# MuMuJun97/semantic_slam_mapping

Measured on AMD Instinct MI355X. Metric: frames/sec semantic-mapping, 640x480 RGB-D, higher is better.
Workload: dtype u8; 1 GPU; configs[1]: synthetic 640x480 RGB-D + precomputed 12-class masks, 1k frames per GPU, ORB 1000 kp/frame, 5 ref frames, leaf 0.10 m; frames_per_gpu=1000, frames_all_gpus=1000, batch_frames=250, matcher_halo_frames=0, parallelism=single GPU

## Files before the change

semantic_slam_mapping_amd/csrc/kernels_match.hip:

```cpp
#include "ssm_internal.h"

#define MT 512
#define TCH 1024

#define QPL 2
__device__ __forceinline__ uint32_t bcnt_acc(uint32_t x, uint32_t acc)
{
    uint32_t r;
    asm("v_bcnt_u32_b32 %0, %1, %2" : "=v"(r) : "v"(x), "v"(acc));
    return r;
}
__device__ __forceinline__ uint32_t umed3(uint32_t a, uint32_t b, uint32_t c)
{
    uint32_t r;
    asm("v_med3_u32 %0, %1, %2, %3" : "=v"(r) : "v"(a), "v"(b), "v"(c));
    return r;
}
template <int T>
__device__ __forceinline__ void match_pair(const uint8_t* __restrict__ q, int nq, const uint8_t* __restrict__ t, int nt,
                                           double ratio, int cap, ssm_dmatch* __restrict__ out, int32_t* __restrict__ nout,
                                           int32_t* __restrict__ knn_idx, int32_t* __restrict__ knn_dist,
                                           int qb = 0, int qe = -1, int32_t* __restrict__ pend = nullptr, int role = 0)
{
    __shared__ uint4 tr[TCH * 2];
    __shared__ int wcnt[T / 64];
    __shared__ int base;
    const int tid = threadIdx.x, lane = tid & 63, wv = tid >> 6;
    if (qe < 0) qe = nq;
    if (tid == 0) base = role == 2 ? qb : 0;
    for (int q0 = qb; q0 < qe; q0 += T * QPL) {
        uint4 a[QPL], b[QPL]; uint32_t k0[QPL], k1[QPL];
#pragma unroll
        for (int u = 0; u < QPL; u++) {
// ... 90 lines not shown
__global__ void __launch_bounds__(MT / 2)
match_seq_kernel(const uint8_t* __restrict__ desc, const int32_t* __restrict__ nkp, int f0, int R, int hist, double ratio, int cap,
                 ssm_dmatch* __restrict__ out, int32_t* __restrict__ nout, int32_t* __restrict__ pend)
{
    const int f = f0 + blockIdx.y, r = blockIdx.x >> 1, half = blockIdx.x & 1;
    const int cur = hist + f, ref = cur - R + r;
    const int slot = f * R + r;
    const int nq = ref >= 0 ? nkp[ref] : -1, nt = nkp[cur];
    if (nq < 0 || nt < 2) { if (threadIdx.x == 0 && half == 0) nout[slot] = -1; return; }
    const int split = min(nq, (((nq + 1) >> 1) + 63) & ~63);
    match_pair<MT / 2>(desc + (size_t)ref * cap * 32, nq, desc + (size_t)cur * cap * 32, nt, ratio, cap,
                       out + (size_t)slot * cap, nout + slot, nullptr, nullptr, half ? split : 0, half ? nq : split, pend + blockIdx.y * R + r, half + 1);
}
hipError_t k_match_seq(const uint8_t* desc, const int32_t* nkp, int f0, int n, int R, int hist, double ratio, int cap,
                       ssm_dmatch* out, int32_t* nout, int32_t* pend, hipStream_t s)
{
    hipError_t e = hipMemsetAsync(pend, 0xFF, sizeof(int32_t) * (size_t)n * R, s);
    if (e != hipSuccess) return e;
    match_seq_kernel<<<dim3(2 * R, n), MT / 2, 0, s>>>(desc, nkp, f0, R, hist, ratio, cap, out, nout, pend);
    return hipGetLastError();
}

typedef int v4i __attribute__((ext_vector_type(4)));
typedef int v8i __attribute__((ext_vector_type(8)));
typedef float v16f __attribute__((ext_vector_type(16)));
typedef __attribute__((address_space(3))) void* lds_ptr_t;
#define MM_QB 256
#define MM_DB SSM_MATCH_DESC_BYTES
#define MM_KS 4
#define MM_TILE (32 * MM_DB)
#ifndef MM_ABLATE
#define MM_ABLATE 0
#endif

__global__ void __launch_bounds__(256)
match_expand_kernel(const uint8_t* __restrict__ desc, const int32_t* __restrict__ nkp, int row0, int cap, int capT,
                    uint8_t* __restrict__ eq, uint8_t* __restrict__ et)
{
    const int row = row0 + blockIdx.y;
    const int i = blockIdx.x * 256 + threadIdx.x;
    if (i >= capT * 8) return;
    const int r = i & 31, c = (i >> 5) & 7, d = (i >> 8) * 32 + r;
    uint32_t bits = 0;
    if (d < nkp[row]) bits = *reinterpret_cast<const uint32_t*>(desc + ((size_t)row * cap + d) * 32 + 4 * c);
    uint32_t q[4], t[4];
#pragma unroll
    for (int k = 0; k < 4; k++) {
        uint32_t v = (bits >> (8 * k)) & 255u;
        v = (v | (v << 12)) & 0x000F000Fu;
        v = (v | (v << 6)) & 0x03030303u;
        v = (v | (v << 3)) & 0x11111111u;
        q[k] = (v << 3) + 0x22222222u;
        t[k] = (v << 3) ^ 0xAAAAAAAAu;
    }
    const size_t o = (size_t)row * capT * MM_DB + (size_t)i * 16;
    *reinterpret_cast<uint4*>(eq + o) = make_uint4(q[0], q[1], q[2], q[3]);
    *reinterpret_cast<uint4*>(et + o) = make_uint4(t[0], t[1], t[2], t[3]);
}

__device__ __forceinline__ void mm_merge2(uint32_t& a0, uint32_t& a1, uint32_t b0, uint32_t b1)
{
    const uint32_t m = max(a0, b0);
    a0 = min(a0, b0);
    a1 = min(min(m, a1), b1);
}
__device__ __forceinline__ void mm_track(const v16f& acc, uint32_t t32, uint32_t& g0, uint32_t& g1)
{
    float l0 = __builtin_fminf(acc[0], acc[1]), l1 = __builtin_fmaxf(acc[0], acc[1]);
#pragma unroll
    for (int i = 2; i < 16; i++) { l1 = __builtin_amdgcn_fmed3f(acc[i], l0, l1); l0 = __builtin_fminf(acc[i], l0); }
    const uint32_t k0 = (uint32_t)l0, k1 = (uint32_t)l1;
    const uint32_t G0 = ((k0 >> 5) << 16) | ((k0 & 31u) | t32), G1 = ((k1 >> 5) << 16) | ((k1 & 31u) | t32);
    mm_merge2(g0, g1, G0, G1);
}

__global__ void __launch_bounds__(256, 2)
match_mfma_kernel(const uint8_t* __restrict__ eq, const uint8_t* __restrict__ et, const int32_t* __restrict__ nkp,
                  int f0, int n, int R, int hist, int capT, int qblocks, int frames_per_xcd, uint2* __restrict__ knn)
{
    __shared__ __attribute__((aligned(16))) uint4 ring0[MM_TILE / 16];
    __shared__ __attribute__((aligned(16))) uint4 ring1[MM_TILE / 16];
    __shared__ __attribute__((aligned(16))) uint4 ring2[MM_TILE / 16];
    __shared__ __attribute__((aligned(16))) uint4 ring3[MM_TILE / 16];
    const int Y = R * qblocks, xcd = blockIdx.x & 7, j = blockIdx.x >> 3;
    const int frame = xcd * frames_per_xcd + j / Y, y = j % Y;
    if (frame >= n) return;
    const int r = y / qblocks, qb = y - r * qblocks;
    const int f = f0 + frame, cur = hist + f, ref = cur - R + r;
    const int nq = ref >= 0 ? nkp[ref] : -1, nt = nkp[cur];
    if (nq < 0 || nt < 2 || qb * MM_QB >= nq) return;
    const int tid = threadIdx.x, lane = tid & 63, wv = tid >> 6, h = lane >> 5;
    const int q0 = qb * MM_QB + wv * 64;
    v4i b[2][MM_KS];
    {
        const uint4* qp = reinterpret_cast<const uint4*>(eq + ((size_t)ref * capT + q0) * MM_DB) + lane;
#pragma unroll
        for (int u = 0; u < 2; u++)
#pragma unroll
            for (int s = 0; s < MM_KS; s++) {
                uint4 v = make_uint4(0, 0, 0, 0);
                if (q0 + u * 32 < capT) v = qp[(u * MM_TILE + s * 1024) / 16];
                b[u][s] = v4i{(int)v.x, (int)v.y, (int)v.z, (int)v.w};
            }
    }
    v16f cc;
#pragma unroll
    for (int i = 0; i < 16; i++) cc[i] = (float)(4096 + (i & 3) + 8 * (i >> 2) + 4 * h);
    const int ntile = (nt + 31) >> 5;
    uint32_t g0[2] = {0xFFFFFFFFu, 0xFFFFFFFFu}, g1[2] = {0xFFFFFFFFu, 0xFFFFFFFFu};
    const auto rsT = __builtin_amdgcn_make_buffer_rsrc((void*)(et + (size_t)cur * capT * MM_DB), 0, (unsigned)capT * MM_DB, 0x00020000);
    const int wvu = __builtin_amdgcn_readfirstlane(wv);
    auto dma = [&](int T, uint4* ring) {
        if (MM_ABLATE & 4) return;
        const unsigned o = (unsigned)min(T, ntile - 1) * MM_TILE + (unsigned)(wvu * 64 + lane) * 16u;
        __builtin_amdgcn_raw_ptr_buffer_load_lds(rsT, (lds_ptr_t)&ring[wvu * 64], 16, o, 0, 0, 0);
    };
    auto frags = [&](const uint4* buf, v4i (&a)[MM_KS]) {
#pragma unroll
        for (int s = 0; s < MM_KS; s++) { const uint4 v = buf[s * 64 + lane]; a[s] = v4i{(int)v.x, (int)v.y, (int)v.z, (int)v.w}; }
    };
    auto mfma4 = [](const v4i& a, const v4i& bq, const v16f& c) {
        const v8i a8 = {a[0], a[1], a[2], a[3], 0, 0, 0, 0}, b8 = {bq[0], bq[1], bq[2], bq[3], 0, 0, 0, 0};
        return __builtin_amdgcn_mfma_scale_f32_32x32x64_f8f6f4(a8, b8, c, 4, 4, 0, 0x83838383, 0, 0x7F7F7F7F);
    };
    auto issue = [&](const v4i (&a)[MM_KS], v16f& x0, v16f& x1) {
        if (MM_ABLATE & 8) { x0 = cc; x1 = cc; for (int s = 0; s < MM_KS; s++) { x0[s] += (float)a[s][0]; x1[s] += (float)a[s][1]; } return; }
        x0 = mfma4(a[0], b[0][0], cc);
        x1 = mfma4(a[0], b[1][0], cc);
#pragma unroll
        for (int s = 1; s < MM_KS; s++) {
            x0 = mfma4(a[s], b[0][s], x0);
            x1 = mfma4(a[s], b[1][s], x1);
        }
    };
    auto interleave = [&]() {
#pragma unroll
        for (int i = 0; i < 2 * MM_KS; i++) { __builtin_amdgcn_sched_group_barrier(0x008, 1, 0); __builtin_amdgcn_sched_group_barrier(0x002, 12, 0); }
    };
    auto track = [&](const v16f& x0, const v16f& x1, int T) {
        if (MM_ABLATE & 1) { g0[0] = min(g0[0], __float_as_uint(x0[0])); g0[1] = min(g0[1], __float_as_uint(x1[0])); return; }
        mm_track(x0, (uint32_t)T << 5, g0[0], g1[0]); mm_track(x1, (uint32_t)T << 5, g0[1], g1[1]);
    };
    auto track_last = [&](v16f x0, v16f x1, int T) {
        const int valid = nt - T * 32;
#pragma unroll
        for (int i = 0; i < 16; i++) if ((i & 3) + 8 * (i >> 2) + 4 * h >= valid) { x0[i] = 1048576.0f; x1[i] = 1048576.0f; }
        track(x0, x1, T);
    };
#define MM_STEP(T_, rd_, wr_, acur, anxt, xn0, xn1, TRACK) { \
        __builtin_amdgcn_s_waitcnt((MM_ABLATE & 4) ? 0x007F : 0x0072);     \
        if (!(MM_ABLATE & 2)) __builtin_amdgcn_s_barrier();               \
        frags(rd_, anxt); \
        dma((T_) + 4, wr_); \
        __builtin_amdgcn_sched_barrier(0); \
        issue(acur, xn0, xn1); TRACK; interleave(); \
        __builtin_amdgcn_sched_barrier(0); }
    v16f A0, A1, B0, B1;
    v4i aA[MM_KS], aB[MM_KS];
    dma(0, ring0); dma(1, ring1); dma(2, ring2); dma(3, ring3);
    if (!(MM_ABLATE & 4)) __builtin_amdgcn_s_waitcnt(0x0F73);
    if (!(MM_ABLATE & 2)) __builtin_amdgcn_s_barrier();
    frags(ring0, aA);
    MM_STEP(0, ring1, ring0, aA, aB, A0, A1, (void)0)
    int T = 1;
    for (; T + 3 < ntile; T += 4) {
        MM_STEP(T, ring2, ring1, aB, aA, B0, B1, track(A0, A1, T - 1))
        MM_STEP(T + 1, ring3, ring2, aA, aB, A0, A1, track(B0, B1, T))
        MM_STEP(T + 2, ring0, ring3, aB, aA, B0, B1, track(A0, A1, T + 1))
        MM_STEP(T + 3, ring1, ring0, aA, aB, A0, A1, track(B0, B1, T + 2))
    }
    if (T < ntile) MM_STEP(T, ring2, ring1, aB, aA, B0, B1, track(A0, A1, T - 1))
    if (T + 1 < ntile) MM_STEP(T + 1, ring3, ring2, aA, aB, A0, A1, track(B0, B1, T))
    if (T + 2 < ntile) MM_STEP(T + 2, ring0, ring3, aB, aA, B0, B1, track(A0, A1, T + 1))
#undef MM_STEP
    if ((ntile - 1) & 1) track_last(B0, B1, ntile - 1); else track_last(A0, A1, ntile - 1);
    __builtin_amdgcn_s_waitcnt(0x0070);
#pragma unroll
    for (int u = 0; u < 2; u++) {
        const uint32_t o0 = __shfl_xor(g0[u], 32), o1 = __shfl_xor(g1[u], 32);
        const uint32_t m = max(g0[u], o0);
        g0[u] = min(g0[u], o0);
        g1[u] = min(min(m, g1[u]), o1);
    }
    const uint32_t k0 = h ? g0[1] : g0[0], k1 = h ? g1[1] : g1[0];
    const int qi = q0 + lane;
    const int slot = f * R + r;
    if (qi < nq) knn[(size_t)slot * capT + qi] = make_uint2(k0, k1);
}

__global__ void __launch_bounds__(256)
match_compact_kernel(const uint2* __restrict__ knn, const int32_t* __restrict__ nkp, int f0, int R, int hist, int capT, double ratio, int cap,
                     ssm_dmatch* __restrict__ out, int32_t* __restrict__ nout)
{
    __shared__ int wcnt[4];
    const int slot = (f0 + blockIdx.x / R) * R + blockIdx.x % R;
    const int cur = hist + f0 + blockIdx.x / R, ref = cur - R + blockIdx.x % R;
    const int nq = ref >= 0 ? nkp[ref] : -1, nt = nkp[cur];
    const int tid = threadIdx.x, lane = tid & 63, wv = tid >> 6;
    if (nq < 0 || nt < 2) { if (tid == 0) nout[slot] = -1; return; }
    const uint2* kk = knn + (size_t)slot * capT;
    ssm_dmatch* o = out + (size_t)slot * cap;
    int base = 0;
    for (int q0 = 0; q0 < nq; q0 += 256) {
        const int qi = q0 + tid;
        uint2 k = make_uint2(0, 0);
        if (qi < nq) k = kk[qi];
        const int d0 = k.x >> 16, i0 = k.x & 0xFFFF, d1 = k.y >> 16;
        const bool keep = (qi < nq) && ((double)(float)d0 < ratio * (double)(float)d1);
        const unsigned long long bal = __ballot(keep);
        if (lane == 0) wcnt[wv] = __popcll(bal);
        __syncthreads();
        int off = base;
        for (int w = 0; w < wv; w++) off += wcnt[w];
        if (keep) {
            const int kpos = off + __popcll(bal & ((1ull << lane) - 1ull));
            if (kpos < cap) { ssm_dmatch mm; mm.queryIdx = qi; mm.trainIdx = i0; mm.imgIdx = 0; mm.distance = (float)d0; o[kpos] = mm; }
        }
        base += wcnt[0] + wcnt[1] + wcnt[2] + wcnt[3];
        __syncthreads();
    }
    if (tid == 0) nout[slot] = base;
}
hipError_t k_match_expand(const uint8_t* desc, const int32_t* nkp, int row0, int nrows, int cap, int capT, uint8_t* eq, uint8_t* et, hipStream_t s)
{
    if (nrows <= 0) return hipSuccess;
    match_expand_kernel<<<dim3((capT * 8 + 255) / 256, nrows), 256, 0, s>>>(desc, nkp, row0, cap, capT, eq, et);
    return hipGetLastError();
}
hipError_t k_match_seq_mfma(const uint8_t* eq, const uint8_t* et, const int32_t* nkp, int f0, int n, int R, int hist, double ratio, int cap, int capT,
                            void* knn, ssm_dmatch* out, int32_t* nout, hipStream_t s)
{
    const int qblocks = (capT + MM_QB - 1) / MM_QB;
    const int fpx = (n + 7) >> 3;
    match_mfma_kernel<<<8 * fpx * R * qblocks, 256, 0, s>>>(eq, et, nkp, f0, n, R, hist, capT, qblocks, fpx, reinterpret_cast<uint2*>(knn));
    match_compact_kernel<<<n * R, 256, 0, s>>>(reinterpret_cast<const uint2*>(knn), nkp, f0, R, hist, capT, ratio, cap, out, nout);
    return hipGetLastError();
}
```

semantic_slam_mapping_amd/csrc/ssm_abi.hip:

```cpp
#include "ssm_ctx.h"
#include "ssm_host.h"
#include <set>

static const int8_t k_default_pattern[1024] = {
#include "orb_pattern.inc"
};
thread_local std::string g_create_err;
int host_fail(ssm_ctx* c, int code, const std::string& msg) { if (c) c->err = msg; else g_create_err = msg; return code; }
std::unique_lock<std::mutex> host_lock(ssm_ctx* c) { return c ? std::unique_lock<std::mutex>(c->mu) : std::unique_lock<std::mutex>(); }

int ensure_scratch(ssm_ctx* c, size_t bytes, DevBuf<uint8_t>* buf)
{
    DevBuf<uint8_t>& b = buf ? *buf : c->d_scratch;
    if (bytes <= b.bytes()) return SSM_OK;
    if (b) hipStreamSynchronize(c->main.stream);
    return b.alloc(c, bytes);
}
int ensure_pinned(ssm_ctx* c, size_t bytes)
{
    if (bytes <= c->h_pinned.bytes()) return SSM_OK;
    if (c->h_pinned) hipStreamSynchronize(c->main.stream);
    if (c->h_pinned.alloc(c, bytes)) FAIL(c, SSM_E_HIP, "hipHostMalloc failed");
    return SSM_OK;
}
void prof_begin(ssm_ctx* c, hipStream_t s, const char* name)
{
    if (!c->profiling) return;
    auto get = [&]() -> hipEvent_t { if (c->pool_used == c->pool.size()) { c->pool.emplace_back(); (void)c->pool.back().ensure(true); } return c->pool[c->pool_used++]; };
    StageRec r; r.name = name; r.a = get(); r.b = get();
    hipEventRecord(r.a, s);
    c->recs.push_back(r);
}
void prof_end(ssm_ctx* c, hipStream_t s) { if (c->profiling) hipEventRecord(c->recs.back().b, s); }
void prof_reset(ssm_ctx* c) { if (c->profiling) { c->recs.clear(); c->pool_used = 0; } }
// ... 288 lines not shown
    }
    int rc = SSM_OK;
    const hipError_t e = hipStreamSynchronize(c->main.stream);
    if (e != hipSuccess) { c->err = std::string("hipStreamSynchronize: ") + hipGetErrorString(e); rc = SSM_E_HIP; }
    std::vector<std::function<int(ssm_ctx*)>> fins; fins.swap(c->pending);
    for (auto& f : fins) { if (rc == SSM_OK) { const int r = f(c); if (r != SSM_OK) rc = r; } }
    c->h_ring_off = 0; c->d_ring_off = 0;
    return rc;
}
static int ring_take(ssm_ctx* c, size_t hbytes, size_t dbytes, uint8_t** hp, uint8_t** dp)
{
    hbytes = up256(hbytes); dbytes = up256(dbytes);
    if (c->h_ring_off + hbytes > c->d_ring.bytes() || c->d_ring_off + dbytes > c->d_ring.bytes()) {
        int r = wait_pending(c); if (r) return r;
        const size_t need = hbytes > dbytes ? hbytes : dbytes;
        if (need > c->d_ring.bytes()) {
            HIPCHK(c, hipStreamSynchronize(c->main.stream));
            c->h_ring.reset(); c->d_ring.reset();
            const size_t nb = need * 4 > ((size_t)8 << 20) ? need * 4 : ((size_t)8 << 20);
            if (c->h_ring.alloc(c, nb)) FAIL(c, SSM_E_HIP, "hipHostMalloc of the staging ring failed");
            if (c->d_ring.alloc(c, nb)) { c->h_ring.reset(); FAIL(c, SSM_E_HIP, "hipMalloc of the result ring failed"); }
        }
        if (c->h_ring_off + hbytes > c->d_ring.bytes() || c->d_ring_off + dbytes > c->d_ring.bytes()) FAIL(c, SSM_E_HIP, "staging ring: the request does not fit after the wait");
    }
    *hp = c->h_ring + c->h_ring_off; *dp = c->d_ring + c->d_ring_off;
    c->h_ring_off += hbytes; c->d_ring_off += dbytes;
    return SSM_OK;
}
struct OrbBlock {
    size_t kps, desc, pos, bytes;
    explicit OrbBlock(int ocap) : kps(64), desc(kps + (size_t)ocap * sizeof(ssm_keypoint)), pos(desc + (size_t)ocap * 32), bytes(pos + (size_t)ocap * 12) {}
};
static int match_capT(int cap) { return (cap + 31) & ~31; }
static size_t match_exp_bytes(size_t rows, int capT) { return rows * capT * SSM_MATCH_DESC_BYTES; }
static size_t match_knn_bytes(size_t pairs, int capT) { return pairs * capT * 8; }
struct MatchBlock {
    static constexpr size_t counts_bytes = 128, res_hdr = 256;
    int rows, nref, capm, capT;
    size_t rowb, inb, expb, knnb, resb;
    size_t counts, h_res, hbytes;
    size_t d_eq, d_et, d_knn, d_res, dbytes;
    MatchBlock(int rows_, int capm_) : rows(rows_), nref(rows_ - 1), capm(capm_), capT(match_capT(capm_))
    {
        rowb = (size_t)capm * 32; counts = rows * rowb; inb = counts + counts_bytes;
        expb = match_exp_bytes(rows, capT); knnb = up256(match_knn_bytes(nref, capT)); resb = list(nref);
        h_res = (inb + 63) & ~(size_t)63; hbytes = h_res + (resb > knnb ? resb : knnb);
        d_eq = up256(inb); d_et = d_eq + expb; d_knn = d_et + expb; d_res = d_knn + knnb; dbytes = d_res + resb;
    }
    size_t list(int i) const { return res_hdr + (size_t)i * capm * sizeof(ssm_dmatch); }
};
static int orb_extract_enqueue(ssm_ctx* c, const uint8_t* img, int w, int h, int stride, int channels, const uint16_t* depth,
                               ssm_keypoint* kps, uint8_t* desc, float* pos3d, int cap, int* n_out, bool in_place = false)
{
    if (!img || !kps || !desc || !n_out) FAIL(c, SSM_E_INVAL, "null argument");
    if (w != c->g.W || h != c->g.H) FAIL(c, SSM_E_INVAL, "frame size differs from the context configuration");
    if (channels != 1 && channels != 3) FAIL(c, SSM_E_INVAL, "channels must be 1 or 3");
    if (stride < w * channels) FAIL(c, SSM_E_INVAL, "stride smaller than a row");
    const int ocap = c->g.cap;
    const size_t row = (size_t)w * channels, ib = row * h, db = depth ? (size_t)w * h * 2 : 0;
    const OrbBlock B(ocap);
    uint8_t *hp, *dp;
    int r = ring_take(c, ib + db + 64 + B.bytes, B.bytes, &hp, &dp); if (r) return r;
    uint8_t* h_in = hp; uint8_t* h_out = hp + ((ib + db + 63) & ~(size_t)63);
    const bool img_direct = in_place && (size_t)stride == row && host_is_pinned(img), depth_direct = in_place && depth && host_is_pinned(depth);
    if (img_direct) HIPCHK(c, hipMemcpyAsync(c->d_in_img, img, ib, hipMemcpyHostToDevice, c->main.stream));
    else {
// ... 35 lines not shown
    if (!c) return SSM_E_INVAL;
    std::lock_guard<std::mutex> lk(c->mu); hipSetDevice(c->device);
    return orb_extract_enqueue(c, img, w, h, stride, channels, depth, kps, desc, pos3d, cap, n_out);
}
extern "C" int ssm_orb_extract(ssm_ctx* c, const uint8_t* img, int w, int h, int stride, int channels, const uint16_t* depth,
                               ssm_keypoint* kps, uint8_t* desc, float* pos3d, int cap, int* n_out)
{
    if (!c) return SSM_E_INVAL;
    std::lock_guard<std::mutex> lk(c->mu); hipSetDevice(c->device);
    int r = orb_extract_enqueue(c, img, w, h, stride, channels, depth, kps, desc, pos3d, cap, n_out, true); if (r) return r;
    return wait_pending(c);
}
extern "C" int ssm_wait(ssm_ctx* c)
{
    if (!c) return SSM_E_INVAL;
    std::lock_guard<std::mutex> lk(c->mu); hipSetDevice(c->device);
    return wait_pending(c);
}

static int match_mfma_enqueue(ssm_ctx* c, const uint8_t* const* qs, const int* nqs, int nref, const uint8_t* t, int nt, int capm, double ratio,
                              ssm_dmatch* const* outs, const int* caps, int* n_outs, int32_t* idx = nullptr, int32_t* dist = nullptr)
{
    const MatchBlock L(nref + 1, capm);
    uint8_t *hp, *dp;
    int r = ring_take(c, L.hbytes, L.dbytes, &hp, &dp); if (r) return r;
    int32_t hn[MatchBlock::counts_bytes / 4] = {0};
    for (int i = 0; i < nref; i++) { if (nqs[i]) memcpy(hp + i * L.rowb, qs[i], (size_t)nqs[i] * 32); hn[i] = nqs[i]; }
    memcpy(hp + nref * L.rowb, t, (size_t)nt * 32); hn[nref] = nt;
    memcpy(hp + L.counts, hn, sizeof(hn));
    const int32_t* dnk = reinterpret_cast<const int32_t*>(dp + L.counts);
    uint8_t* h_res = hp + L.h_res;
    HIPCHK(c, hipMemcpyAsync(dp, hp, L.inb, hipMemcpyHostToDevice, c->main.stream));
    HIPCHK(c, k_match_expand(dp, dnk, 0, L.rows, capm, L.capT, dp + L.d_eq, dp + L.d_et, c->main.stream));
    HIPCHK(c, k_match_seq_mfma(dp + L.d_eq, dp + L.d_et, dnk, 0, 1, nref, nref, ratio, capm, L.capT, dp + L.d_knn,
                               reinterpret_cast<ssm_dmatch*>(dp + L.d_res + L.list(0)), reinterpret_cast<int32_t*>(dp + L.d_res), c->main.stream));
    if (idx) {
        const int nq = nqs[0];
        HIPCHK(c, hipMemcpyAsync(h_res, dp + L.d_knn, (size_t)nq * 8, hipMemcpyDeviceToHost, c->main.stream));
        c->pending.push_back([=](ssm_ctx*) -> int {
            const uint2* hk = reinterpret_cast<const uint2*>(h_res);
            for (int i = 0; i < nq; i++) { idx[2*i] = hk[i].x & 0xFFFF; idx[2*i+1] = hk[i].y & 0xFFFF; dist[2*i] = hk[i].x >> 16; dist[2*i+1] = hk[i].y >> 16; }
            return SSM_OK;
        });
        return SSM_OK;
    }
    HIPCHK(c, hipMemcpyAsync(h_res, dp + L.d_res, L.list(nref - 1) + (size_t)nqs[nref - 1] * sizeof(ssm_dmatch), hipMemcpyDeviceToHost, c->main.stream));
    struct { ssm_dmatch* out[16]; int cap[16]; } to;
    for (int i = 0; i < nref; i++) { to.out[i] = outs[i]; to.cap[i] = caps[i]; }
    c->pending.push_back([=](ssm_ctx* cc) -> int {
        for (int i = 0; i < nref; i++) {
            int32_t n; memcpy(&n, h_res + 4 * (size_t)i, 4);
            if (n < 0) n = 0;
            n_outs[i] = n;
            if (n > to.cap[i]) FAIL(cc, SSM_E_CAPACITY, "match buffer too small (need " + std::to_string(n) + ")");
            memcpy(to.out[i], h_res + L.list(i), sizeof(ssm_dmatch) * (size_t)n);
        }
        return SSM_OK;
    });
    return SSM_OK;
}
static int match_valu(ssm_ctx* c, const uint8_t* q, int nq, const uint8_t* t, int nt, double ratio, int32_t* idx, int32_t* dist, ssm_dmatch* out, int cap, int* n_out)
{
    const bool want_knn = idx != nullptr;
    const size_t need = (size_t)(nq + nt) * 32 + sizeof(MatchPair) + (size_t)nq * (16 + 16) + 64;
    int r = ensure_scratch(c, need); if (r) return r;
    uint8_t* dd = c->d_scratch;
    ssm_dmatch* dm = reinterpret_cast<ssm_dmatch*>(dd + (size_t)(nq + nt) * 32);
    int32_t* di = reinterpret_cast<int32_t*>(dm + nq); int32_t* ds = di + 2 * (size_t)nq;
    MatchPair* dp = reinterpret_cast<MatchPair*>(ds + 2 * (size_t)nq); int32_t* dn = reinterpret_cast<int32_t*>(dp + 1);
    MatchPair p; p.qoff = 0; p.nq = nq; p.toff = nq; p.nt = nt; p.out_slot = 0;
    HIPCHK(c, hipMemcpyAsync(dd, q, (size_t)nq * 32, hipMemcpyHostToDevice, c->main.stream));
    HIPCHK(c, hipMemcpyAsync(dd + (size_t)nq * 32, t, (size_t)nt * 32, hipMemcpyHostToDevice, c->main.stream));
    HIPCHK(c, hipMemcpyAsync(dp, &p, sizeof(p), hipMemcpyHostToDevice, c->main.stream));
    HIPCHK(c, k_match_pairs(dd, dp, 1, ratio, nq, dm, dn, want_knn ? di : nullptr, want_knn ? ds : nullptr, c->main.stream));
    int n = 0;
    HIPCHK(c, hipMemcpyAsync(&n, dn, 4, hipMemcpyDeviceToHost, c->main.stream));
    HIPCHK(c, hipStreamSynchronize(c->main.stream));
    if (want_knn) {
        HIPCHK(c, hipMemcpy(idx, di, (size_t)nq * 8, hipMemcpyDeviceToHost));
        HIPCHK(c, hipMemcpy(dist, ds, (size_t)nq * 8, hipMemcpyDeviceToHost));
    } else {
        *n_out = n;
        if (n > cap) FAIL(c, SSM_E_CAPACITY, "match buffer too small (need " + std::to_string(n) + ")");
        HIPCHK(c, hipMemcpy(out, dm, sizeof(ssm_dmatch) * n, hipMemcpyDeviceToHost));
    }
    return SSM_OK;
}
static int match_host(ssm_ctx* c, const uint8_t* q, int nq, const uint8_t* t, int nt, double ratio, int32_t* idx, int32_t* dist, ssm_dmatch* out, int cap, int* n_out)
{
    if (nq < 0 || nt < 0 || (nq && !q) || (nt && !t)) FAIL(c, SSM_E_INVAL, "bad descriptor arguments");
    if (nt < 2) FAIL(c, SSM_E_TOO_FEW_TRAIN, "knnMatch(k=2) needs at least 2 train descriptors");
    if (nt > 65535) FAIL(c, SSM_E_INVAL, "at most 65535 train descriptors per call");
    if (nq == 0) { if (n_out) *n_out = 0; return SSM_OK; }
    if (!c->match_mfma) return match_valu(c, q, nq, t, nt, ratio, idx, dist, out, cap, n_out);
    return match_mfma_enqueue(c, &q, &nq, 1, t, nt, nq > nt ? nq : nt, ratio, &out, &cap, n_out, idx, dist);
}
extern "C" int ssm_hamming_knn2(ssm_ctx* c, const uint8_t* q, int nq, const uint8_t* t, int nt, int32_t* idx, int32_t* dist)
{
    if (!c) return SSM_E_INVAL;
    std::lock_guard<std::mutex> lk(c->mu); hipSetDevice(c->device);
    if (nq > 0 && (!idx || !dist)) FAIL(c, SSM_E_INVAL, "null output");
    int r = match_host(c, q, nq, t, nt, c->cfg.knn_match_ratio, idx, dist, nullptr, 0, nullptr); if (r) return r;
    return wait_pending(c);
}
extern "C" int ssm_match(ssm_ctx* c, const uint8_t* q, int nq, const uint8_t* t, int nt, double ratio, ssm_dmatch* out, int cap, int* n_out)
{
    if (!c) return SSM_E_INVAL;
    std::lock_guard<std::mutex> lk(c->mu); hipSetDevice(c->device);
    if (!n_out || (cap > 0 && !out)) FAIL(c, SSM_E_INVAL, "null output");
    int r = match_host(c, q, nq, t, nt, ratio, nullptr, nullptr, out, cap, n_out); if (r) return r;
    return wait_pending(c);
}
extern "C" int ssm_match_async(ssm_ctx* c, const uint8_t* q, int nq, const uint8_t* t, int nt, double ratio, ssm_dmatch* out, int cap, int* n_out)
{
    if (!c) return SSM_E_INVAL;
    std::lock_guard<std::mutex> lk(c->mu); hipSetDevice(c->device);
    if (!n_out || (cap > 0 && !out)) FAIL(c, SSM_E_INVAL, "null output");
    return match_host(c, q, nq, t, nt, ratio, nullptr, nullptr, out, cap, n_out);
}
static int match_refs_enqueue(ssm_ctx* c, const uint8_t* const* refs, const int* nrefs, int nref, const uint8_t* cur, int ncur, double ratio,
                              ssm_dmatch* const* outs, const int* caps, int* n_outs)
{
    if (nref < 0 || (nref && (!refs || !nrefs || !outs || !caps || !n_outs)) || ncur < 0 || (ncur && !cur)) FAIL(c, SSM_E_INVAL, "bad arguments");
    if (nref == 0) return SSM_OK;
    if (ncur < 2) FAIL(c, SSM_E_TOO_FEW_TRAIN, "knnMatch(k=2) needs at least 2 train descriptors");
    if (ncur > 65535) FAIL(c, SSM_E_INVAL, "at most 65535 train descriptors per call");
    int capm = ncur;
    for (int i = 0; i < nref; i++) { if (nrefs[i] < 0 || (nrefs[i] && !refs[i]) || (caps[i] > 0 && !outs[i])) FAIL(c, SSM_E_INVAL, "bad reference set"); if (nrefs[i] > capm) capm = nrefs[i]; }
    if (c->match_mfma && nref <= 16) return match_mfma_enqueue(c, refs, nrefs, nref, cur, ncur, capm, ratio, outs, caps, n_outs);
    for (int i = 0; i < nref; i++) {
        if (nrefs[i] == 0) { n_outs[i] = 0; continue; }
        int r = match_host(c, refs[i], nrefs[i], cur, ncur, ratio, nullptr, nullptr, outs[i], caps[i], &n_outs[i]); if (r) return r;
    }
    return SSM_OK;
}
extern "C" int ssm_match_refs_async(ssm_ctx* c, const uint8_t* const* refs, const int* nrefs, int nref, const uint8_t* cur, int ncur, double ratio,
                                    ssm_dmatch* const* outs, const int* caps, int* n_outs)
{
    if (!c) return SSM_E_INVAL;
    std::lock_guard<std::mutex> lk(c->mu); hipSetDevice(c->device);
    return match_refs_enqueue(c, refs, nrefs, nref, cur, ncur, ratio, outs, caps, n_outs);
}
extern "C" int ssm_match_refs(ssm_ctx* c, const uint8_t* const* refs, const int* nrefs, int nref, const uint8_t* cur, int ncur, double ratio,
                              ssm_dmatch* const* outs, const int* caps, int* n_outs)
{
    if (!c) return SSM_E_INVAL;
    std::lock_guard<std::mutex> lk(c->mu); hipSetDevice(c->device);
    int r = match_refs_enqueue(c, refs, nrefs, nref, cur, ncur, ratio, outs, caps, n_outs); if (r) return r;
    return wait_pending(c);
}

extern "C" int ssm_moving_mask(ssm_ctx* c, const uint8_t* sem, int w, int h, int stride, uint8_t* mask)
{
    if (!c) return SSM_E_INVAL;
    std::lock_guard<std::mutex> lk(c->mu); hipSetDevice(c->device);
    if (!sem || !mask) FAIL(c, SSM_E_INVAL, "null argument");
    if (w != c->g.W || h != c->g.H) FAIL(c, SSM_E_INVAL, "frame size differs from the context configuration");
    if (stride < w * 3) FAIL(c, SSM_E_INVAL, "stride smaller than a row");
    HIPCHK(c, hipMemcpy2DAsync(c->d_in_sem, (size_t)w * 3, sem, stride, (size_t)w * 3, h, hipMemcpyHostToDevice, c->main.stream));
    HIPCHK(c, k_moving_mask(c->d_in_sem, 1, w, h, c->d_mask, c->main.stream));
    HIPCHK(c, hipMemcpyAsync(mask, c->d_mask, (size_t)w * h, hipMemcpyDeviceToHost, c->main.stream));
    HIPCHK(c, hipStreamSynchronize(c->main.stream));
// ... 50 lines not shown
    DALLOC(c, nd, (size_t)(n + R) * g.cap * 32); DALLOC(c, nn, (size_t)(n + R));
    if (!c->d_hist_tmp) DALLOC(c, c->d_hist_tmp, (size_t)R * g.cap * 32 + (size_t)R * 4);
    if (c->d_desc_all && c->prev_n >= 0) {
        HIPCHK(c, hipMemcpy(nd, c->d_desc_all, (size_t)(c->prev_n + R) * g.cap * 32, hipMemcpyDeviceToDevice));
        HIPCHK(c, hipMemcpy(nn, c->d_nkp_all, (size_t)(c->prev_n + R) * 4, hipMemcpyDeviceToDevice));
    }
    c->d_desc_all = std::move(nd); c->d_nkp_all = std::move(nn); c->seq_cap = n;
    return SSM_OK;
}
extern "C" int ssm_seq_process(ssm_ctx* c, const ssm_frames_dev* in, ssm_seq_out_dev* out)
{
    if (!c) return SSM_E_INVAL;
    std::lock_guard<std::mutex> lk(c->mu); hipSetDevice(c->device);
    if (!in || in->n < 0) FAIL(c, SSM_E_INVAL, "bad arguments");
    const int stages = in->stages ? in->stages : (SSM_STAGE_ORB | SSM_STAGE_MATCH | SSM_STAGE_MAP);
    if ((stages & (SSM_STAGE_ORB | SSM_STAGE_MATCH)) && !in->bgr) FAIL(c, SSM_E_INVAL, "bgr is required");
    if ((stages & SSM_STAGE_MAP) && (!in->depth || !in->bgr || (!in->sem_bgr && !(stages & SSM_STAGE_SEGNET)))) FAIL(c, SSM_E_INVAL, "bgr, depth and sem_bgr (or SSM_STAGE_SEGNET) are required for the map stage");
    const OrbGeom& g = c->g; const int R = c->R, n = in->n, W = g.W, H = g.H; const hipStream_t s = c->main.stream;
    const size_t npix = (size_t)W * H;
    if (c->gov.unexamined) { const int r0 = map_settle(c, c->mapdev.tail ? c->mapdev.tail : c->main.stream, 0); if (r0) return r0; }
    int r = ensure_seq(c, n > 0 ? n : 1); if (r) return r;
    c->recs.clear(); c->pool_used = 0;
    const size_t row = (size_t)g.cap * 32;
    if (in->continue_sequence && c->prev_n >= 0) {
        int32_t* tn = reinterpret_cast<int32_t*>(c->d_hist_tmp + (size_t)R * row);
        HIPCHK(c, hipMemcpyAsync(c->d_hist_tmp, c->d_desc_all + (size_t)c->prev_n * row, (size_t)R * row, hipMemcpyDeviceToDevice, s));
        HIPCHK(c, hipMemcpyAsync(tn, c->d_nkp_all + c->prev_n, (size_t)R * 4, hipMemcpyDeviceToDevice, s));
        HIPCHK(c, hipMemcpyAsync(c->d_desc_all, c->d_hist_tmp, (size_t)R * row, hipMemcpyDeviceToDevice, s));
        HIPCHK(c, hipMemcpyAsync(c->d_nkp_all, tn, (size_t)R * 4, hipMemcpyDeviceToDevice, s));
    } else {
        HIPCHK(c, hipMemsetAsync(c->d_nkp_all, 0xFF, (size_t)R * 4, s));
    }
    uint8_t* desc = c->d_desc_all + (size_t)R * row; int32_t* nkp = c->d_nkp_all + R;
    const bool mfma = c->match_mfma && (stages & SSM_STAGE_MATCH);
    if (mfma) HIPCHK(c, k_match_expand(c->d_desc_all, c->d_nkp_all, 0, R, g.cap, c->capT, c->d_exp_q, c->d_exp_t, s));
    const bool side_work = (stages & (SSM_STAGE_MAP | SSM_STAGE_SEGNET)) != 0;
    const bool two_chains = !c->serialize && !(stages & SSM_STAGE_SEGNET) && n > c->B && (stages & SSM_STAGE_ORB) && (W & 15) == 0;
    const bool side = side_work && !c->serialize && !two_chains;
    if (side || two_chains) { r = ensure_side_streams(c); if (r) return r; }
    if (two_chains) { r = ensure_alt(c); if (r) return r; }
    const int nch = two_chains ? (n > 2 * c->B ? 3 : 2) : 1;
    const bool map3 = two_chains && c->mapdev.own_stream == 1;
    Lane* const used[3] = {&c->side[0], nch == 3 ? &c->side[2] : nullptr, map3 ? &c->side[1] : nullptr};
    if (side || two_chains) { r = lanes_fork(c, {used[0], used[1], used[2]}); if (r) return r; }
    int bi = 0;
    for (int f0 = 0; f0 < n; f0 += c->B, bi++) {
        const int nb = (n - f0 < c->B) ? n - f0 : c->B;
        const int chain = bi % nch;
        OrbChain& ch = c->chain[chain]; const hipStream_t cs = ch.lane->stream; OrbWork& work = ch.work;
        auto front = [&]() -> int {
            if (stages & SSM_STAGE_ORB) {
                r = run_orb(c, cs, work, in->bgr + (size_t)f0 * npix * 3, 3, in->depth ? in->depth + (size_t)f0 * npix : nullptr, nb,
                            c->d_kps + (size_t)f0 * g.cap, desc + (size_t)f0 * row, c->d_pos3d + (size_t)f0 * g.cap * 3, nkp + f0);
                if (r) return r;
                if (mfma) { prof_begin(c, cs, "match"); HIPCHK(c, k_match_expand(c->d_desc_all, c->d_nkp_all, R + f0, nb, g.cap, c->capT, c->d_exp_q, c->d_exp_t, cs)); prof_end(c, cs); }
                if (two_chains) {
                    HIPCHK(c, hipEventRecord(ch.orb_done, cs));
                    for (int k = 1; k < nch && k <= bi; k++) HIPCHK(c, hipStreamWaitEvent(cs, c->chain[(bi - k) % nch].orb_done, 0));
                }
            }
            if (stages & SSM_STAGE_MATCH) {
                prof_begin(c, cs, "match");
                if (mfma) {
                    if (!(stages & SSM_STAGE_ORB)) HIPCHK(c, k_match_expand(c->d_desc_all, c->d_nkp_all, R + f0, nb, g.cap, c->capT, c->d_exp_q, c->d_exp_t, cs));
                    HIPCHK(c, k_match_seq_mfma(c->d_exp_q, c->d_exp_t, c->d_nkp_all, f0, nb, R, R, c->cfg.knn_match_ratio, g.cap, c->capT, c->d_knn, c->d_matches, c->d_nmatch, cs));
                } else
                    HIPCHK(c, k_match_seq(c->d_desc_all, c->d_nkp_all, f0, nb, R, R, c->cfg.knn_match_ratio, g.cap, c->d_matches, c->d_nmatch, c->d_match_pend + (size_t)f0 * R, cs));
                prof_end(c, cs);
            }
            return SSM_OK;
        };
        auto back = [&]() -> int {
            if (!side_work) return SSM_OK;
            Lane& ml = map3 ? c->side[1] : side ? c->side[0] : *ch.lane;
            const hipStream_t s = ml.stream;
            const uint8_t* sem_src = in->sem_bgr ? in->sem_bgr + (size_t)f0 * npix * 3 : nullptr;
            if (stages & SSM_STAGE_SEGNET) {
                r = seg_init(c); if (r) return r;
                prof_begin(c, s, "segnet");
                r = seg_forward_dev(c, ml, in->bgr + (size_t)f0 * npix * 3, nb, nullptr, c->seg->d_sem_gen, 0); if (r) return r;
                prof_end(c, s);
                sem_src = c->seg->d_sem_gen;
            }
            for (int q0 = 0, nq; (stages & SSM_STAGE_MAP) && q0 < nb; q0 += nq) {
                r = map_before_launch(c, s, nb - q0, &nq); if (r) return r;
                const int g0 = f0 + q0;
                const uint8_t* sem_q = sem_src + (size_t)q0 * npix * 3;
                if ((W & 15) == 0) {
                    prof_begin(c, s, "map_fuse");
                    { MapLaunch L; L.depth = in->depth + (size_t)g0 * npix; L.rgb = in->bgr + (size_t)g0 * npix * 3; L.sem = sem_q; L.pose = in->pose ? in->pose + (size_t)g0 * 16 : nullptr;
                      L.n = nq; L.w = W; L.h = H; L.npoints = c->d_npoints + g0;
                      r = map_fuse_launch(c, s, L); if (r) return r; }
                    prof_end(c, s);
                } else {
                    prof_begin(c, s, "mask");
                    HIPCHK(c, k_moving_mask(sem_q, nq, W, H, c->d_mask, s)); prof_end(c, s);
                    prof_begin(c, s, "backproject");
                    HIPCHK(c, k_backproject(in->depth + (size_t)g0 * npix, in->bgr + (size_t)g0 * npix * 3, sem_q, c->d_mask,
// ... 104 lines not shown
```

semantic_slam_mapping_amd/csrc/ssm_internal.h:

```cpp
#pragma once
#include <hip/hip_runtime.h>
#include <stdint.h>
#include <vector>
#include "../../include/ssm_hip.h"
#include "ssm_orb_plan.h"
#include "cloud_table.h"

#define SSM_VOX_EMPTY ((int64_t)-1)
inline size_t up256(size_t v) { return (v + 255) & ~(size_t)255; }
struct Carve {
    size_t off = 0; template <class T> size_t take(size_t count, size_t align = 256) { const size_t at = (off + align - 1) & ~(align - 1); off = at + count * sizeof(T); return at; }
    size_t end() { return take<uint8_t>(0); }
};

typedef uint2 cand_t;

struct DeviceInfo { int id = 0, cus = 256, max_lds = 160 * 1024; };
hipError_t allow_dynamic_lds(const void* fn, size_t bytes, int limit);

hipError_t k_gray(const uint8_t* img, int channels, int n, const OrbGeom& g, uint8_t* pyr, hipStream_t s);
hipError_t k_copy_gray_strided(const uint8_t* img, int stride, const OrbGeom& g, uint8_t* pyr, hipStream_t s);
hipError_t k_pyramid(int n, const OrbGeom& g, uint8_t* pyr, const int32_t* const* xofs, const int16_t* const* xa,
                     const int32_t* const* yofs, const int16_t* const* ya, const void* const* xgroups, hipStream_t s);
hipError_t k_pyramid_bands(const uint8_t* img, int channels, int n, const OrbGeom& g, uint8_t* pyr, const PyrBandPlan& p,
                           const int32_t* const* yofs, const int16_t* const* ya, const void* const* xgroups, const void* const* xgroups8, hipStream_t s);
hipError_t k_blur(int n, const OrbGeom& g, const uint8_t* pyr, uint8_t* blur, hipStream_t s);
hipError_t k_blur_mfma(int n, const OrbGeom& g, const uint8_t* pyr, uint8_t* blur, const void* tab, hipStream_t s);
hipError_t k_fast(int n, const OrbGeom& g, const uint8_t* pyr, cand_t* cand, int32_t* ncand, int32_t* cellmax , hipStream_t s);
size_t k_fast_ncand_pad(int nframes, const OrbGeom& g);
size_t k_fast_cellmax_ints(int nframes, const OrbGeom& g);
hipError_t k_octree(int n, const OrbGeom& g, const cand_t* cand, const int32_t* ncand, const int32_t* cellmax, uint16_t* node_of,
                    uint32_t* sel, int32_t* nsel, int32_t* status, hipStream_t s);
hipError_t k_describe(int n, const OrbGeom& g, const uint8_t* pyr, const uint8_t* blur, const uint32_t* sel,
                      const int32_t* nsel, const float* pattern_f , const uint16_t* depth, ssm_camera cam, void* kpaux ,
                      ssm_keypoint* kps, uint8_t* desc, float* pos3d, int32_t* nkp, hipStream_t s);

struct MatchPair { int32_t qoff, nq, toff, nt, out_slot; };
hipError_t k_match_pairs(const uint8_t* desc, const MatchPair* pairs, int npairs, double ratio, int cap,
                         ssm_dmatch* out, int32_t* nout, int32_t* knn_idx, int32_t* knn_dist, hipStream_t s);
hipError_t k_match_seq(const uint8_t* desc, const int32_t* nkp, int f0, int n, int R, int hist, double ratio, int cap,
                       ssm_dmatch* out, int32_t* nout, int32_t* pend , hipStream_t s);

#define SSM_MATCH_DESC_BYTES 128
hipError_t k_match_expand(const uint8_t* desc, const int32_t* nkp, int row0, int nrows, int cap, int capT, uint8_t* eq, uint8_t* et, hipStream_t s);
hipError_t k_match_seq_mfma(const uint8_t* eq, const uint8_t* et, const int32_t* nkp, int f0, int n, int R, int hist, double ratio, int cap, int capT,
                            void* knn , ssm_dmatch* out, int32_t* nout, hipStream_t s);

hipError_t k_moving_mask(const uint8_t* sem, int n, int w, int h, uint8_t* mask, hipStream_t s);
hipError_t k_backproject(const uint16_t* depth, const uint8_t* rgb, const uint8_t* sem, const uint8_t* mask,
                         const double* pose, int n, int w, int h, ssm_camera cam, double max_distance,
                         int32_t* chunk_cnt, int64_t* chunk_off, int32_t* npoints, int64_t* total,
                         ssm_point* out, hipStream_t s);
int backproject_chunks(int w, int h);

hipError_t k_voxel_clear(ssm_voxel* tab, int cap_log2, int32_t* counters, hipStream_t s);
hipError_t k_voxel_insert(const ssm_point* pts, const int64_t* n_dev, int64_t n_max, float leaf, ssm_voxel* tab,
                          int cap_log2, int32_t* counters, hipStream_t s);
struct MapDiv { double rscale, rfx, rfy; };
bool k_map_div(const ssm_camera& cam, MapDiv& md);
hipError_t k_map_fuse(const uint16_t* depth, const uint8_t* rgb, const uint8_t* sem, const double* pose, int n, int w, int h,
                      ssm_camera cam, const MapDiv& md, bool exact, double max_distance, float leaf,
                      ssm_voxel* tab, int cap_log2, int32_t* counters, int32_t* npoints, hipStream_t s, int32_t* skip, int hw, int tag, const int32_t* redo_ids, int nredo);
int k_map_fuse_blocks_per_frame(int w, int h);
int k_map_fuse_block_records(void);
int k_map_fuse_resident_blocks(void);
int k_map_fuse_skip_cap(void);
hipError_t k_voxel_merge(const ssm_voxel* src, int n, ssm_voxel* tab, int cap_log2, int32_t* counters, hipStream_t s);
hipError_t k_voxel_rehash(const ssm_voxel* src, int src_cap_log2, ssm_voxel* tab, int cap_log2, int32_t* counters, hipStream_t s);
hipError_t k_voxel_compact(const ssm_voxel* tab, int cap_log2, ssm_voxel* out, int32_t* n_out, hipStream_t s);
hipError_t k_voxel_gather_points(const ssm_voxel* compact, const uint32_t* order, int n, ssm_point* out, hipStream_t s);
hipError_t k_voxel_gather_table(const ssm_voxel* compact, const uint32_t* order, int n, ssm_voxel* out, hipStream_t s);
hipError_t k_voxel_bounds(const ssm_point* pts, int n, float* minmax6, hipStream_t s);
hipError_t k_cloud_transform(const ssm_point* src, int n, const double* T, ssm_point* dst, hipStream_t s);
hipError_t voxel_sort_pairs(void* tmp, size_t* tmp_bytes, const ssm_voxel* compact, int n, uint64_t* keys_a, uint64_t* keys_b,
                            uint32_t* idx_a, uint32_t* idx_b, hipStream_t s);

hipError_t k_synth(uint64_t seed, int first, int n, int w, int h, uint8_t* bgr, uint16_t* depth, uint8_t* sem,
                   uint8_t* lab, double* pose, hipStream_t s);

// ... 127 lines not shown
```

Baseline: 188,700 frames/s.

## Encode train index into MFMA accumulator scale and track top-2 in float

Rescales the MFMA block scale so the Hamming distance sits in the high bits of the float accumulator and the train column index in the low bits. Each tile then only needs float min/med3 ops to track the best two candidates, with a per-tile offset subtraction instead of integer packing. The integer key is rebuilt once at the end. The scheduling group size for VALU ops between MFMAs drops from 12 to 7, and a capT bound check falls back to the VALU matcher for oversized sets. Precision limits on exact float representation are the main correctness risk.

```diff
diff --git a/semantic_slam_mapping_amd/csrc/kernels_match.hip b/semantic_slam_mapping_amd/csrc/kernels_match.hip
--- a/semantic_slam_mapping_amd/csrc/kernels_match.hip
+++ b/semantic_slam_mapping_amd/csrc/kernels_match.hip
@@ -1,4 +1,5 @@
 #include "ssm_internal.h"
+#include "match_keys.h"
 
 #define MT 512
 #define TCH 1024
@@ -155,6 +156,9 @@
 #ifndef MM_ABLATE
 #define MM_ABLATE 0
 #endif
+#ifndef MM_VPM
+#define MM_VPM 7
+#endif
 
 __global__ void __launch_bounds__(256)
 match_expand_kernel(const uint8_t* __restrict__ desc, const int32_t* __restrict__ nkp, int row0, int cap, int capT,
@@ -181,25 +185,25 @@
     *reinterpret_cast<uint4*>(et + o) = make_uint4(t[0], t[1], t[2], t[3]);
 }
 
-__device__ __forceinline__ void mm_merge2(uint32_t& a0, uint32_t& a1, uint32_t b0, uint32_t b1)
-{
-    const uint32_t m = max(a0, b0);
-    a0 = min(a0, b0);
-    a1 = min(min(m, a1), b1);
-}
-__device__ __forceinline__ void mm_track(const v16f& acc, uint32_t t32, uint32_t& g0, uint32_t& g1)
-{
-    float l0 = __builtin_fminf(acc[0], acc[1]), l1 = __builtin_fmaxf(acc[0], acc[1]);
-#pragma unroll
-    for (int i = 2; i < 16; i++) { l1 = __builtin_amdgcn_fmed3f(acc[i], l0, l1); l0 = __builtin_fminf(acc[i], l0); }
-    const uint32_t k0 = (uint32_t)l0, k1 = (uint32_t)l1;
-    const uint32_t G0 = ((k0 >> 5) << 16) | ((k0 & 31u) | t32), G1 = ((k1 >> 5) << 16) | ((k1 & 31u) | t32);
-    mm_merge2(g0, g1, G0, G1);
+__device__ __forceinline__ void mm_merge2(float& a0, float& a1, float b0, float b1)
+{
+    const float m = __builtin_fmaxf(a0, b0);
+    a0 = __builtin_fminf(a0, b0);
+    a1 = __builtin_fminf(__builtin_fminf(m, a1), b1);
+}
+__device__ __forceinline__ void mm_track(const v16f& acc, float& l0, float& l1)
+{
+    l0 -= 32.0f; l1 -= 32.0f;
+#pragma unroll
+    for (int i = 0; i < 16; i += 2) {
+        l1 = __builtin_fminf(__builtin_amdgcn_fmed3f(acc[i], acc[i + 1], l0), l1);
+        l0 = __builtin_fminf(__builtin_fminf(acc[i], acc[i + 1]), l0);
+    }
 }
 
 __global__ void __launch_bounds__(256, 2)
 match_mfma_kernel(const uint8_t* __restrict__ eq, const uint8_t* __restrict__ et, const int32_t* __restrict__ nkp,
-                  int f0, int n, int R, int hist, int capT, int qblocks, int frames_per_xcd, uint2* __restrict__ knn)
+                  int f0, int n, int R, int hist, int capT, int qblocks, int frames_per_xcd, int e, uint2* __restrict__ knn)
 {
     __shared__ __attribute__((aligned(16))) uint4 ring0[MM_TILE / 16];
     __shared__ __attribute__((aligned(16))) uint4 ring1[MM_TILE / 16];
@@ -228,9 +232,10 @@
     }
     v16f cc;
 #pragma unroll
-    for (int i = 0; i < 16; i++) cc[i] = (float)(4096 + (i & 3) + 8 * (i >> 2) + 4 * h);
+    for (int i = 0; i < 16; i++) cc[i] = (float)(match_key_c0(e) + (i & 3) + 8 * (i >> 2) + 4 * h);
+    const int scale_t = (127 + e) * 0x01010101;
     const int ntile = (nt + 31) >> 5;
-    uint32_t g0[2] = {0xFFFFFFFFu, 0xFFFFFFFFu}, g1[2] = {0xFFFFFFFFu, 0xFFFFFFFFu};
+    float l0[2] = {SSM_MATCH_KEY_BIG, SSM_MATCH_KEY_BIG}, l1[2] = {SSM_MATCH_KEY_BIG, SSM_MATCH_KEY_BIG};
     const auto rsT = __builtin_amdgcn_make_buffer_rsrc((void*)(et + (size_t)cur * capT * MM_DB), 0, (unsigned)capT * MM_DB, 0x00020000);
     const int wvu = __builtin_amdgcn_readfirstlane(wv);
     auto dma = [&](int T, uint4* ring) {
@@ -242,9 +247,9 @@
 #pragma unroll
         for (int s = 0; s < MM_KS; s++) { const uint4 v = buf[s * 64 + lane]; a[s] = v4i{(int)v.x, (int)v.y, (int)v.z, (int)v.w}; }
     };
-    auto mfma4 = [](const v4i& a, const v4i& bq, const v16f& c) {
+    auto mfma4 = [scale_t](const v4i& a, const v4i& bq, const v16f& c) {
         const v8i a8 = {a[0], a[1], a[2], a[3], 0, 0, 0, 0}, b8 = {bq[0], bq[1], bq[2], bq[3], 0, 0, 0, 0};
-        return __builtin_amdgcn_mfma_scale_f32_32x32x64_f8f6f4(a8, b8, c, 4, 4, 0, 0x83838383, 0, 0x7F7F7F7F);
+        return __builtin_amdgcn_mfma_scale_f32_32x32x64_f8f6f4(a8, b8, c, 4, 4, 0, scale_t, 0, 0x7F7F7F7F);
     };
     auto issue = [&](const v4i (&a)[MM_KS], v16f& x0, v16f& x1) {
         if (MM_ABLATE & 8) { x0 = cc; x1 = cc; for (int s = 0; s < MM_KS; s++) { x0[s] += (float)a[s][0]; x1[s] += (float)a[s][1]; } return; }
@@ -258,16 +263,16 @@
     };
     auto interleave = [&]() {
 #pragma unroll
-        for (int i = 0; i < 2 * MM_KS; i++) { __builtin_amdgcn_sched_group_barrier(0x008, 1, 0); __builtin_amdgcn_sched_group_barrier(0x002, 12, 0); }
+        for (int i = 0; i < 2 * MM_KS; i++) { __builtin_amdgcn_sched_group_barrier(0x008, 1, 0); __builtin_amdgcn_sched_group_barrier(0x002, MM_VPM, 0); }
     };
     auto track = [&](const v16f& x0, const v16f& x1, int T) {
-        if (MM_ABLATE & 1) { g0[0] = min(g0[0], __float_as_uint(x0[0])); g0[1] = min(g0[1], __float_as_uint(x1[0])); return; }
-        mm_track(x0, (uint32_t)T << 5, g0[0], g1[0]); mm_track(x1, (uint32_t)T << 5, g0[1], g1[1]);
+        if (MM_ABLATE & 1) { l0[0] = __builtin_fminf(l0[0], x0[0]); l0[1] = __builtin_fminf(l0[1], x1[0]); return; }
+        mm_track(x0, l0[0], l1[0]); mm_track(x1, l0[1], l1[1]);
     };
     auto track_last = [&](v16f x0, v16f x1, int T) {
         const int valid = nt - T * 32;
 #pragma unroll
-        for (int i = 0; i < 16; i++) if ((i & 3) + 8 * (i >> 2) + 4 * h >= valid) { x0[i] = 1048576.0f; x1[i] = 1048576.0f; }
+        for (int i = 0; i < 16; i++) if ((i & 3) + 8 * (i >> 2) + 4 * h >= valid) { x0[i] = SSM_MATCH_KEY_BIG; x1[i] = SSM_MATCH_KEY_BIG; }
         track(x0, x1, T);
     };
 #define MM_STEP(T_, rd_, wr_, acur, anxt, xn0, xn1, TRACK) { \
@@ -299,13 +304,11 @@
     if ((ntile - 1) & 1) track_last(B0, B1, ntile - 1); else track_last(A0, A1, ntile - 1);
     __builtin_amdgcn_s_waitcnt(0x0070);
 #pragma unroll
-    for (int u = 0; u < 2; u++) {
-        const uint32_t o0 = __shfl_xor(g0[u], 32), o1 = __shfl_xor(g1[u], 32);
-        const uint32_t m = max(g0[u], o0);
-        g0[u] = min(g0[u], o0);
-        g1[u] = min(min(m, g1[u]), o1);
-    }
-    const uint32_t k0 = h ? g0[1] : g0[0], k1 = h ? g1[1] : g1[0];
+    for (int u = 0; u < 2; u++) mm_merge2(l0[u], l1[u], __shfl_xor(l0[u], 32), __shfl_xor(l1[u], 32));
+    const float back = (float)(32 * (ntile - 1));
+    const uint32_t c0 = (uint32_t)((h ? l0[1] : l0[0]) + back), c1 = (uint32_t)((h ? l1[1] : l1[0]) + back);
+    const uint32_t imask = (2u << e) - 1u;
+    const uint32_t k0 = ((c0 >> (e + 1)) << 16) | (c0 & imask), k1 = ((c1 >> (e + 1)) << 16) | (c1 & imask);
     const int qi = q0 + lane;
     const int slot = f * R + r;
     if (qi < nq) knn[(size_t)slot * capT + qi] = make_uint2(k0, k1);
@@ -351,11 +354,12 @@
     return hipGetLastError();
 }
 hipError_t k_match_seq_mfma(const uint8_t* eq, const uint8_t* et, const int32_t* nkp, int f0, int n, int R, int hist, double ratio, int cap, int capT,
-                            void* knn, ssm_dmatch* out, int32_t* nout, hipStream_t s)
-{
+                            int e, void* knn, ssm_dmatch* out, int32_t* nout, hipStream_t s)
+{
+    if (e < 0 || e != match_key_exp(capT)) return hipErrorInvalidValue;
     const int qblocks = (capT + MM_QB - 1) / MM_QB;
     const int fpx = (n + 7) >> 3;
-    match_mfma_kernel<<<8 * fpx * R * qblocks, 256, 0, s>>>(eq, et, nkp, f0, n, R, hist, capT, qblocks, fpx, reinterpret_cast<uint2*>(knn));
+    match_mfma_kernel<<<8 * fpx * R * qblocks, 256, 0, s>>>(eq, et, nkp, f0, n, R, hist, capT, qblocks, fpx, e, reinterpret_cast<uint2*>(knn));
     match_compact_kernel<<<n * R, 256, 0, s>>>(reinterpret_cast<const uint2*>(knn), nkp, f0, R, hist, capT, ratio, cap, out, nout);
     return hipGetLastError();
 }
diff --git a/semantic_slam_mapping_amd/csrc/match_keys.h b/semantic_slam_mapping_amd/csrc/match_keys.h
--- /dev/null
+++ b/semantic_slam_mapping_amd/csrc/match_keys.h
@@ -0,0 +1,16 @@
+#pragma once
+
+#define SSM_MATCH_KEY_MAX_CAPT 32768
+#define SSM_MATCH_KEY_BIG 1e30f
+
+constexpr int match_key_exp(int capT)
+{
+    if (capT < 1 || capT > SSM_MATCH_KEY_MAX_CAPT) return -1;
+    int e = 4;
+    while ((2 << e) < capT) e++;
+    return e;
+}
+constexpr bool match_key_fits(int capT) { return match_key_exp(capT) >= 0; }
+constexpr int match_key_c0(int e) { return 1 << (e + 8); }
+constexpr int match_key_max(int e, int capT) { return (256 << (e + 1)) + capT - 1; }
+constexpr int match_key_sum_bound(int e) { return 512 * (1 << e) + 31; }
diff --git a/semantic_slam_mapping_amd/csrc/ssm_abi.hip b/semantic_slam_mapping_amd/csrc/ssm_abi.hip
--- a/semantic_slam_mapping_amd/csrc/ssm_abi.hip
+++ b/semantic_slam_mapping_amd/csrc/ssm_abi.hip
@@ -1,5 +1,6 @@
 #include "ssm_ctx.h"
 #include "ssm_host.h"
+#include "match_keys.h"
 #include <set>
 
 static const int8_t k_default_pattern[1024] = {
@@ -354,6 +355,7 @@
     explicit OrbBlock(int ocap) : kps(64), desc(kps + (size_t)ocap * sizeof(ssm_keypoint)), pos(desc + (size_t)ocap * 32), bytes(pos + (size_t)ocap * 12) {}
 };
 static int match_capT(int cap) { return (cap + 31) & ~31; }
+static bool match_mfma_fits(int cap) { return match_key_fits(match_capT(cap)); }
 static size_t match_exp_bytes(size_t rows, int capT) { return rows * capT * SSM_MATCH_DESC_BYTES; }
 static size_t match_knn_bytes(size_t pairs, int capT) { return pairs * capT * 8; }
 struct MatchBlock {
@@ -455,7 +457,7 @@
     uint8_t* h_res = hp + L.h_res;
     HIPCHK(c, hipMemcpyAsync(dp, hp, L.inb, hipMemcpyHostToDevice, c->main.stream));
     HIPCHK(c, k_match_expand(dp, dnk, 0, L.rows, capm, L.capT, dp + L.d_eq, dp + L.d_et, c->main.stream));
-    HIPCHK(c, k_match_seq_mfma(dp + L.d_eq, dp + L.d_et, dnk, 0, 1, nref, nref, ratio, capm, L.capT, dp + L.d_knn,
+    HIPCHK(c, k_match_seq_mfma(dp + L.d_eq, dp + L.d_et, dnk, 0, 1, nref, nref, ratio, capm, L.capT, match_key_exp(L.capT), dp + L.d_knn,
                                reinterpret_cast<ssm_dmatch*>(dp + L.d_res + L.list(0)), reinterpret_cast<int32_t*>(dp + L.d_res), c->main.stream));
     if (idx) {
         const int nq = nqs[0];
@@ -515,7 +517,7 @@
     if (nt < 2) FAIL(c, SSM_E_TOO_FEW_TRAIN, "knnMatch(k=2) needs at least 2 train descriptors");
     if (nt > 65535) FAIL(c, SSM_E_INVAL, "at most 65535 train descriptors per call");
     if (nq == 0) { if (n_out) *n_out = 0; return SSM_OK; }
-    if (!c->match_mfma) return match_valu(c, q, nq, t, nt, ratio, idx, dist, out, cap, n_out);
+    if (!c->match_mfma || !match_mfma_fits(nq > nt ? nq : nt)) return match_valu(c, q, nq, t, nt, ratio, idx, dist, out, cap, n_out);
     return match_mfma_enqueue(c, &q, &nq, 1, t, nt, nq > nt ? nq : nt, ratio, &out, &cap, n_out, idx, dist);
 }
 extern "C" int ssm_hamming_knn2(ssm_ctx* c, const uint8_t* q, int nq, const uint8_t* t, int nt, int32_t* idx, int32_t* dist)
@@ -550,7 +552,7 @@
     if (ncur > 65535) FAIL(c, SSM_E_INVAL, "at most 65535 train descriptors per call");
     int capm = ncur;
     for (int i = 0; i < nref; i++) { if (nrefs[i] < 0 || (nrefs[i] && !refs[i]) || (caps[i] > 0 && !outs[i])) FAIL(c, SSM_E_INVAL, "bad reference set"); if (nrefs[i] > capm) capm = nrefs[i]; }
-    if (c->match_mfma && nref <= 16) return match_mfma_enqueue(c, refs, nrefs, nref, cur, ncur, capm, ratio, outs, caps, n_outs);
+    if (c->match_mfma && nref <= 16 && match_mfma_fits(capm)) return match_mfma_enqueue(c, refs, nrefs, nref, cur, ncur, capm, ratio, outs, caps, n_outs);
     for (int i = 0; i < nref; i++) {
         if (nrefs[i] == 0) { n_outs[i] = 0; continue; }
         int r = match_host(c, refs[i], nrefs[i], cur, ncur, ratio, nullptr, nullptr, outs[i], caps[i], &n_outs[i]); if (r) return r;
@@ -667,7 +669,7 @@
         HIPCHK(c, hipMemsetAsync(c->d_nkp_all, 0xFF, (size_t)R * 4, s));
     }
     uint8_t* desc = c->d_desc_all + (size_t)R * row; int32_t* nkp = c->d_nkp_all + R;
-    const bool mfma = c->match_mfma && (stages & SSM_STAGE_MATCH);
+    const bool mfma = c->match_mfma && (stages & SSM_STAGE_MATCH) && match_key_fits(c->capT);
     if (mfma) HIPCHK(c, k_match_expand(c->d_desc_all, c->d_nkp_all, 0, R, g.cap, c->capT, c->d_exp_q, c->d_exp_t, s));
     const bool side_work = (stages & (SSM_STAGE_MAP | SSM_STAGE_SEGNET)) != 0;
     const bool two_chains = !c->serialize && !(stages & SSM_STAGE_SEGNET) && n > c->B && (stages & SSM_STAGE_ORB) && (W & 15) == 0;
@@ -698,7 +700,7 @@
                 prof_begin(c, cs, "match");
                 if (mfma) {
                     if (!(stages & SSM_STAGE_ORB)) HIPCHK(c, k_match_expand(c->d_desc_all, c->d_nkp_all, R + f0, nb, g.cap, c->capT, c->d_exp_q, c->d_exp_t, cs));
-                    HIPCHK(c, k_match_seq_mfma(c->d_exp_q, c->d_exp_t, c->d_nkp_all, f0, nb, R, R, c->cfg.knn_match_ratio, g.cap, c->capT, c->d_knn, c->d_matches, c->d_nmatch, cs));
+                    HIPCHK(c, k_match_seq_mfma(c->d_exp_q, c->d_exp_t, c->d_nkp_all, f0, nb, R, R, c->cfg.knn_match_ratio, g.cap, c->capT, match_key_exp(c->capT), c->d_knn, c->d_matches, c->d_nmatch, cs));
                 } else
                     HIPCHK(c, k_match_seq(c->d_desc_all, c->d_nkp_all, f0, nb, R, R, c->cfg.knn_match_ratio, g.cap, c->d_matches, c->d_nmatch, c->d_match_pend + (size_t)f0 * R, cs));
                 prof_end(c, cs);
diff --git a/semantic_slam_mapping_amd/csrc/ssm_internal.h b/semantic_slam_mapping_amd/csrc/ssm_internal.h
--- a/semantic_slam_mapping_amd/csrc/ssm_internal.h
+++ b/semantic_slam_mapping_amd/csrc/ssm_internal.h
@@ -44,7 +44,7 @@
 #define SSM_MATCH_DESC_BYTES 128
 hipError_t k_match_expand(const uint8_t* desc, const int32_t* nkp, int row0, int nrows, int cap, int capT, uint8_t* eq, uint8_t* et, hipStream_t s);
 hipError_t k_match_seq_mfma(const uint8_t* eq, const uint8_t* et, const int32_t* nkp, int f0, int n, int R, int hist, double ratio, int cap, int capT,
-                            void* knn , ssm_dmatch* out, int32_t* nout, hipStream_t s);
+                            int e, void* knn , ssm_dmatch* out, int32_t* nout, hipStream_t s);
 
 hipError_t k_moving_mask(const uint8_t* sem, int n, int w, int h, uint8_t* mask, hipStream_t s);
 hipError_t k_backproject(const uint16_t* depth, const uint8_t* rgb, const uint8_t* sem, const uint8_t* mask,
```

Result: faster. 193,100 frames/s, median of 6 (+2.3%).
